# nekStab/nekStab_next

Hardware: AMD Instinct MI355X
Metric: Arnoldi-step GB/s (achieved HBM) + Ritz-value rel-err, N=1e8 m=128 (higher is better)
Workload: dtype f64

## Files before the change

### include/nekkrylov.h

```cpp
#ifndef NEKKRYLOV_H
#define NEKKRYLOV_H

#include <stddef.h>
#include <stdint.h>

#ifdef __cplusplus
extern "C" {
#endif

#define NKV_ABI_VERSION 3

#define NKV_TILE 4096
#define NKV_MAX_COLS 1024
#define NKV_ROT_MAX_OUT 256

#define NKV_OK 0
#define NKV_EINVAL 1
#define NKV_EHIP 2
#define NKV_ENAN 3
#define NKV_ESHAPE 4
#define NKV_ECALLBACK 5
#define NKV_EBREAKDOWN 6

#define NKV_TIME 0x1u
#define NKV_ACCUMULATE 0x2u
#define NKV_OVERWRITE 0x4u
#define NKV_NORM2 0x8u
#define NKV_TIME_DOT 0x10u
#define NKV_X_IS_LAST 0x20u
#define NKV_MGS2 0x40u
#define NKV_CHECK_BREAKDOWN 0x80u
#define NKV_MGS_ICWY 0x100u
#define NKV_MGS_LAGGED 0x200u
#define NKV_SFD_MONITOR 0x400u
#define NKV_TDF_STORE 0x800u
#define NKV_BF_IMAG 0x1000u
#define NKV_BF_PERTURBATION 0x2000u

typedef struct nkv_layout {
    int64_t n_v;
    int64_t n_p;
    int64_t sv;
    int64_t sp;
    int64_t ld;
    int32_t n_wf;
    int32_t rank0;
} nkv_layout;

int nkv_abi_version(void);
int nkv_layout_init(nkv_layout* L, int ldim, int lx1, int lx2, int64_t nelv, int64_t nelt, int n_scalars,
                    int ifpo, int rank0);
const char* nkv_last_error(void);
int nkv_device_info(int* device, int* cu_count, int64_t* hbm_bytes, char* name, int name_len);
size_t nkv_workspace_bytes(const nkv_layout* L, int max_cols);
int nkv_check_status(void* ws, void* stream);

int nkv_zero(const nkv_layout* L, double* x, unsigned flags, void* stream);
int nkv_copy(const nkv_layout* L, double* dst, const double* src, unsigned flags, void* stream);
int nkv_scal(const nkv_layout* L, double* x, double alpha, unsigned flags, void* stream);
int nkv_axpby(const nkv_layout* L, double* x, double alpha, const double* y, double beta,
// ... 14 lines not shown
                     double* f, double* nrm2_dev, void* ws, unsigned flags, void* stream);
int nkv_block_update_dot(const nkv_layout* L, const double* w, const double* Q, int j, const double* h_dev,
                         double* f, double* hout_dev, void* ws, unsigned flags, void* stream);
int nkv_arnoldi_finish(const nkv_layout* L, const double* f, const double* nrm2_dev, double* q_out,
                       int j, const double* h1_dev, const double* h2_dev, double* hcol_dev,
                       unsigned flags, void* stream);

int nkv_combine(const nkv_layout* L, const double* Q, int k, const double* y_dev, double* out, unsigned flags,
                void* stream);
int nkv_normalize_store(const nkv_layout* L, const double* f, const double* nrm2_dev, double* q_next,
                        double* beta_dev, unsigned flags, void* stream);
int nkv_mgs2_step(const nkv_layout* L, const double* w, const double* Q, int j, double* f, double* q_out,
                  double* hcol_dev, void* ws, unsigned flags, void* stream);
int nkv_axpy_dot(const nkv_layout* L, const double* w, double* f, const double* alpha_dev, const double* qa,
                 const double* qb, double* out_dev, void* ws, unsigned flags, void* stream);

int nkv_block_dot2(const nkv_layout* L, const double* w, const double* Q, int j, const double* x,
                   const double* y, double* h_dev, void* ws, unsigned flags, void* stream);
int nkv_dcgs2_coef(int m, const double* hq_dev, const double* hw_dev, const double* nrm_prev_dev, double* H_dev,
                   int64_t ldh, double* coef_dev, void* ws, void* stream);
int nkv_dcgs2_update(const nkv_layout* L, const double* w, const double* Q, int m, const double* coef_dev,
                     double* qj, const double* win, double* fout, double* nrm2_dev, void* ws, unsigned flags,
                     void* stream);

int nkv_mgs_icwy_solve(int j, double* G, int64_t ldg, const double* grow, const double* b, double* x,
                       void* stream);

int nkv_gkl_coef(int side, int m, const double* hq_dev, const double* hw_dev, double* M_dev, int64_t ldm,
                 double* A_self, double* r_self, const double* A_other, const double* r_other, int64_t lda,
                 double* coef_dev, void* ws, void* stream);

typedef int (*nkv_matvec_fn)(void* user, const double* x, double* y, void* stream);
typedef int (*nkv_allreduce_fn)(void* user, double* buf, int n, void* stream);
size_t nkv_arnoldi_scratch_doubles(int m);
int nkv_arnoldi_dcgs2(const nkv_layout* L, const double* w, double* Q, int mstart, int mend, double* H_dev,
                      int64_t ldh, double* f, double* scratch_dev, void* ws, nkv_matvec_fn matvec, void* mv_user,
                      nkv_allreduce_fn allreduce, void* ar_user, unsigned flags, void* stream);

int nkv_gmres_dcgs2(const nkv_layout* L, const double* w, double* Q, int kmax, double beta, double tol2,
                    double* H_dev, int64_t ldh, double* f, double* scratch_dev, void* ws, nkv_matvec_fn matvec,
                    void* mv_user, nkv_allreduce_fn allreduce, void* ar_user, double* res_hist, int* k_out,
                    unsigned flags, void* stream);

int nkv_update_hessenberg(const nkv_layout* L, const double* w, const double* Q, int j, double* f, double* q_out,
                          double* hcol_dev, double* scratch_dev, void* ws, nkv_allreduce_fn allreduce, void* ar_user,
                          unsigned flags, void* stream);
// ... 129 lines not shown
```

### nekstab_next_amd/_lib.py

```python
from __future__ import annotations

import ctypes
import os
from ctypes import CFUNCTYPE, POINTER, Structure, c_char_p, c_double, c_int, c_int32, c_int64, c_size_t, c_uint, c_uint64, c_void_p

import torch

_HERE = os.path.dirname(os.path.abspath(__file__))
LIB_PATH = os.path.join(_HERE, "libnekkrylov.so")

NKV_ABI_VERSION = 3
NKV_TILE = 4096
NKV_MAX_COLS = 1024
NKV_ROT_MAX_OUT = 256
NKV_GS_MAX_FIELDS = 64
NKV_OK, NKV_EINVAL, NKV_EHIP, NKV_ENAN, NKV_ESHAPE, NKV_ECALLBACK, NKV_EBREAKDOWN = 0, 1, 2, 3, 4, 5, 6
NKV_TIME = 0x1
NKV_ACCUMULATE = 0x2
NKV_OVERWRITE = 0x4
NKV_NORM2 = 0x8
NKV_TIME_DOT = 0x10
NKV_X_IS_LAST = 0x20
NKV_MGS2 = 0x40
NKV_MGS_ICWY = 0x100
NKV_MGS_LAGGED = 0x200
NKV_CHECK_BREAKDOWN = 0x80
NKV_SFD_MONITOR = 0x400
NKV_TDF_STORE = 0x800
NKV_BF_IMAG = 0x1000
NKV_BF_PERTURBATION = 0x2000
(NKV_VC_VORTICITY, NKV_VC_LAMBDA2, NKV_VC_Q, NKV_VC_DELTA, NKV_VC_SWIRLING, NKV_VC_OMEGA, NKV_VC_SYMMETRIC,
 NKV_VC_ASSYMETRIC, NKV_VC_LAMBDA_CI, NKV_VC_COUNT) = range(10)


class NkvError(RuntimeError):

    def __init__(self, code: int, where: str, msg: str):
        super().__init__(f"{where}: status {code}: {msg}")
        self.code = code


class NkvNaNError(NkvError, FloatingPointError):
    """NaN detected in a dot product (reference aborts: core/nek_vectors.f90:108-111)."""


class NkvBreakdownError(NkvError):
    """NKV_CHECK_BREAKDOWN: a one-call factorisation reached an invariant subspace (include/nekkrylov.h)."""


class nkv_layout(Structure):
    _fields_ = [
        ("n_v", c_int64),
        ("n_p", c_int64),
# ... 13 lines not shown
_SIGNATURES = {
    "nkv_abi_version": (c_int, []),
    "nkv_layout_init": (c_int, [_L, c_int, c_int, c_int, c_int64, c_int64, c_int, c_int, c_int]),
    "nkv_last_error": (c_char_p, []),
    "nkv_device_info": (c_int, [POINTER(c_int), POINTER(c_int), POINTER(c_int64), c_char_p, c_int]),
    "nkv_workspace_bytes": (c_size_t, [_L, c_int]),
    "nkv_check_status": (c_int, [_P, _P]),
    "nkv_zero": (c_int, [_L, _P, c_uint, _P]),
    "nkv_copy": (c_int, [_L, _P, _P, c_uint, _P]),
    "nkv_scal": (c_int, [_L, _P, c_double, c_uint, _P]),
    "nkv_axpby": (c_int, [_L, _P, c_double, _P, c_double, c_uint, _P]),
    "nkv_sub3": (c_int, [_L, _P, _P, _P, c_uint, _P]),
    "nkv_axpy_dev": (c_int, [_L, _P, _P, c_double, _P, c_uint, _P]),
    "nkv_normalize_dev": (c_int, [_L, _P, _P, _P, c_uint, _P]),
    "nkv_dot": (c_int, [_L, _P, _P, _P, _P, _P, c_uint, _P]),
    "nkv_block_dot": (c_int, [_L, _P, _P, c_int, _P, _P, _P, c_uint, _P]),
    "nkv_block_update": (c_int, [_L, _P, _P, c_int, _P, _P, _P, _P, c_uint, _P]),
    "nkv_block_update_dot": (c_int, [_L, _P, _P, c_int, _P, _P, _P, _P, c_uint, _P]),
    "nkv_arnoldi_finish": (c_int, [_L, _P, _P, _P, c_int, _P, _P, _P, c_uint, _P]),
    "nkv_block_dot2": (c_int, [_L, _P, _P, c_int, _P, _P, _P, _P, c_uint, _P]),
    "nkv_dcgs2_coef": (c_int, [c_int, _P, _P, _P, _P, c_int64, _P, _P, _P]),
    "nkv_mgs_icwy_solve": (c_int, [c_int, _P, c_int64, _P, _P, _P, _P]),
    "nkv_dcgs2_update": (c_int, [_L, _P, _P, c_int, _P, _P, _P, _P, _P, _P, c_uint, _P]),
    "nkv_arnoldi_scratch_doubles": (c_size_t, [c_int]),
    "nkv_arnoldi_dcgs2": (c_int, [_L, _P, _P, c_int, c_int, _P, c_int64, _P, _P, _P, MATVEC_FN, _P, ALLREDUCE_FN, _P,
                                  c_uint, _P]),
    "nkv_update_hessenberg": (c_int, [_L, _P, _P, c_int, _P, _P, _P, _P, _P, ALLREDUCE_FN, _P, c_uint, _P]),
    "nkv_gmres_dcgs2": (c_int, [_L, _P, _P, c_int, c_double, c_double, _P, c_int64, _P, _P, _P, MATVEC_FN, _P,
                                ALLREDUCE_FN, _P, _P, _P, c_uint, _P]),
    "nkv_arnoldi_factorization": (c_int, [_L, _P, _P, c_int, c_int, _P, c_int64, _P, _P, _P, MATVEC_FN, _P,
                                          ALLREDUCE_FN, _P, c_uint, _P]),
    "nkv_combine": (c_int, [_L, _P, c_int, _P, _P, c_uint, _P]),
    "nkv_normalize_store": (c_int, [_L, _P, _P, _P, _P, c_uint, _P]),
    "nkv_mgs2_step": (c_int, [_L, _P, _P, c_int, _P, _P, _P, _P, c_uint, _P]),
    "nkv_axpy_dot": (c_int, [_L, _P, _P, _P, _P, _P, _P, _P, c_uint, _P]),
    "nkv_rotate": (c_int, [_L, _P, c_int, _P, c_int, _P]),
    "nkv_rotate_cols": (c_int, [_L, _P, c_int, _P, c_int, c_int, _P]),
    "nkv_op_diag": (c_int, [_L, _P, _P, _P, c_double, _P]),
    "nkv_op_rot2": (c_int, [_L, _P, _P, _P, _P, _P, c_int, _P]),
    "nkv_op_cdiag": (c_int, [_L, _P, _P, _P, _P, c_int, _P]),
    "nkv_fill_hash": (c_int, [_L, _P, c_uint64, c_int64, c_int64, _P]),
    "nkv_mth_rand_add": (c_int, [_L, c_int, c_int, c_int, c_int64, _P, _P, _P, c_double, c_double, c_double, _P, _P]),
    "nkv_group_average": (c_int, [c_int64, _P, _P, _P, _P]),
    "nkv_symmetric_seed": (c_int, [_L, _P, _P, c_double, _P, _P, _P, _P]),
    "nkv_gs_pack": (c_int, [c_int, POINTER(c_void_p), c_int64, c_int64, _P, c_int64, _P, _P]),
    "nkv_gs_average": (c_int, [c_int, POINTER(c_void_p), c_int64, c_int64, _P, _P, _P, c_int64, c_int, _P]),
# ... 87 lines not shown
```

### nekstab_next_amd/arnoldi.py

```python
from __future__ import annotations

import numpy as np
import torch

from . import _lib
from ._lib import NKV_NORM2, NKV_TIME, NKV_TIME_DOT, NKV_X_IS_LAST
from .operators import LinearOperator
from .vector import Basis, NekContext, NekVector


class HessenbergDev:

    def __init__(self, ctx: NekContext, k: int):
        self.ctx, self.k = ctx, k
        self.t = torch.zeros((k, k + 1), dtype=torch.float64, device=ctx.device)

    def col_ptr(self, c: int) -> int:
        return self.t[c].data_ptr()

    def download(self) -> np.ndarray:
        return np.asfortranarray(self.t.detach().cpu().numpy().T)

    def upload(self, H: np.ndarray) -> None:
        self.t.copy_(torch.as_tensor(np.ascontiguousarray(np.asarray(H, dtype=np.float64).T)).to(self.ctx.device))
# ... 60 lines not shown
    elif mode == "mgs2":
        ctx.call("nkv_dot", w, f.ptr, Q.col_ptr(0), h1[0:1].data_ptr(), ws, tf, st)
        ctx.comm.allreduce_(h1[0:1])
        fl = NKV_TIME | (NKV_TIME_DOT if tf else 0)
        for p, h in enumerate((h1, h2)):
            for i in range(j):
                last = i + 1 == j
                qn = Q.col_ptr(i + 1) if not last else (Q.col_ptr(0) if p == 0 else None)
                out = h[i + 1:i + 2] if not last else (h2[0:1] if p == 0 else nrm)
                ctx.call("nkv_axpy_dot", w, f.ptr, h[i:i + 1].data_ptr(), Q.col_ptr(i), qn, out.data_ptr(), ws, fl,
                         st)
                ctx.comm.allreduce_(out)
    else:
        raise ValueError(f"unknown orthogonalisation mode {mode!r}")
    if ctx.timer:
        ctx.timer.begin("finish")
    ctx.call("nkv_arnoldi_finish", f.ptr, nrm.data_ptr(), out_ptr, j, h1.data_ptr(), h2.data_ptr(),
             hcol_ptr, 0, st)
    if ctx.timer:
        ctx.timer.end("finish", 16.0 * ctx.layout.N)


def _dcgs2_step(ctx: NekContext, Q: Basis, Hd: HessenbergDev, j: int, f: NekVector, first: bool,
                nrm2: torch.Tensor | None = None) -> None:
    w, ws, st = ctx.w.data_ptr(), ctx.ws.data_ptr(), ctx.stream
    lay, tm = ctx.layout, ctx.timer
    tf = NKV_TIME if ctx.time_in_dot else 0
    m = j - 1
    h = ctx.hd[: 2 * j]
    hp, cp = h.data_ptr(), ctx.coef.data_ptr()
    u = Q.col_ptr(m)
    if tm:
        tm.begin("block_dot2")
    ctx.call("nkv_block_dot2", w, Q.ptr, j, u, f.ptr, hp, ws, tf | NKV_X_IS_LAST, st)
    if tm:
        tm.end("block_dot2", 8.0 * ((j - 1) * lay.N_w + 2 * lay.N_w + lay.n_v))
    ctx.comm.allreduce_(h)
    nprev = None if first else (nrm2.data_ptr() if nrm2 is not None else hp + 8 * m)
    ctx.call_nl("nkv_dcgs2_coef", m, hp, hp + 8 * j, nprev, Hd.t.data_ptr(), Hd.k + 1, cp, ws, st)
    if tm:
        tm.begin("dcgs2_update")
    ctx.call("nkv_dcgs2_update", w, Q.ptr, m, cp, u, f.ptr, Q.col_ptr(j), None if nrm2 is None else nrm2.data_ptr(),
             ws, NKV_TIME | (NKV_TIME_DOT if tf else 0), st)
    if tm:
        tm.end("dcgs2_update", 8.0 * (m * lay.N + 4 * lay.N) + (0.0 if nrm2 is None else 8.0 * lay.n_v))
    if nrm2 is not None:
        ctx.comm.allreduce_(nrm2)


def _dcgs2_close(ctx: NekContext, Q: Basis, Hd: HessenbergDev, m: int) -> None:
    w, ws, st = ctx.w.data_ptr(), ctx.ws.data_ptr(), ctx.stream
    lay, tm = ctx.layout, ctx.timer
    tf = NKV_TIME if ctx.time_in_dot else 0
    h, coef = ctx.hd[: m + 1], ctx.coef
    u = Q.col_ptr(m)
    if tm:
        tm.begin("block_dot")
    ctx.call("nkv_block_dot", w, Q.ptr, m + 1, u, h.data_ptr(), ws, tf, st)
    if tm:
        tm.end("block_dot", 8.0 * ((m + 1) * lay.N_w + lay.N_w + lay.n_v))
    ctx.comm.allreduce_(h)
    ctx.call_nl("nkv_dcgs2_coef", m, h.data_ptr(), None, h.data_ptr() + 8 * m, Hd.t.data_ptr(), Hd.k + 1,
                coef.data_ptr(), ws, st)
    if tm:
        tm.begin("block_update")
    ctx.call("nkv_block_update", w, Q.ptr, m, h.data_ptr(), u, None, ws, NKV_TIME, st)
    if tm:
        tm.end("block_update", 8.0 * (m * lay.N + 2 * lay.N))
    ctx.call("nkv_normalize_dev", u, coef[2 * m + 3:].data_ptr(), None, 0, st)


def _icwy_gram(ctx: NekContext, Q: Basis, mstart: int) -> torch.Tensor:
    ldg = ctx.max_cols + 1
    G = getattr(ctx, "_icwy_G", None)
    if G is None:
        G = ctx._icwy_G = torch.zeros((ldg, ldg), dtype=torch.float64, device=ctx.device)
    w, ws, st = ctx.w.data_ptr(), ctx.ws.data_ptr(), ctx.stream
    tf = NKV_TIME if ctx.time_in_dot else 0
    for i in range(1, mstart - 1):
        ctx.call("nkv_block_dot", w, Q.ptr, i, Q.col_ptr(i), G[i].data_ptr(), ws, tf, st)
        ctx.comm.allreduce_(G[i, :i])
    return G


def _icwy_step(ctx: NekContext, Q: Basis, Hd: HessenbergDev, j: int, f: NekVector, G: torch.Tensor) -> None:
    w, ws, st = ctx.w.data_ptr(), ctx.ws.data_ptr(), ctx.stream
    lay, tm = ctx.layout, ctx.timer
    tf = NKV_TIME if ctx.time_in_dot else 0
    ldg = G.shape[1]
    h = ctx.hd[: 2 * j]
    hp, gp = h.data_ptr(), G.data_ptr()
    h1, h2, nrm = ctx.h1[:j], ctx.h2[:j], ctx.scal[3:4]
# ... 138 lines not shown


def _dcgs2_native(ctx: NekContext, op: LinearOperator, Q: Basis, Hd: HessenbergDev, mstart: int, mend: int,
                  f: NekVector, transpose: bool, entry: str = "nkv_arnoldi_dcgs2", flags: int = 0) -> None:
    lib = ctx.lib
    scratch = _native_scratch(ctx, mend)
    base, ld8, fptr = Q.ptr, 8 * ctx.layout.ld, f.ptr
    apply = op.rmatvec if transpose else op.matvec
    errors = []

    def matvec(_user, x, y, _stream):
        try:
            c, r = divmod((x or 0) - base, ld8)
            if r or not 0 <= c < Q.k or y != fptr:
                raise ValueError(f"{entry} matvec callback: x={x}, y={y} are not a basis column and f")
            apply(Q[c], f)
            return 0
        except BaseException as e:
            errors.append(e)
            return 1

    mv_c = _lib.MATVEC_FN(matvec)
    ar_c = _allreduce_callback(ctx, scratch, errors)
    rc = getattr(lib, entry)(ctx._Lp, ctx.w.data_ptr(), Q.ptr, int(mstart), int(mend), Hd.t.data_ptr(), Hd.k + 1,
                             fptr, scratch.data_ptr(), ctx.ws.data_ptr(), mv_c, None, ar_c, None,
                             (NKV_TIME_DOT if ctx.time_in_dot else 0) | flags, ctx.stream)
    if errors:
        raise errors[0]
    _lib.check(rc, entry)


def arnoldi_factorization(ctx: NekContext, op: LinearOperator, Q: Basis, Hd: HessenbergDev, mstart: int,
                          mend: int, f: NekVector | None = None, mode: str = "cgs2", transpose: bool = False,
                          on_step=None) -> None:
    if mend < mstart:
        return
    if Q.k < mend + 1:
        raise ValueError("basis too small")
    if f is None:
        f = ctx.vector()
    if mode == "dcgs2-native":
        if on_step is None:
            if mend > ctx.max_cols or mend + 1 > Hd.k + 1:
                raise ValueError(f"step {mend} exceeds max_cols {ctx.max_cols} / H size {Hd.k}")
            _dcgs2_native(ctx, op, Q, Hd, mstart, mend, f, transpose)
            return
        mode = "dcgs2"
    if mode == "dcgs2" and on_step is not None:
        if mend > ctx.max_cols or mend + 1 > Hd.k + 1:
            raise ValueError(f"step {mend} exceeds max_cols {ctx.max_cols} / H size {Hd.k}")
        for mstep in range(mstart, mend + 1):
            (op.rmatvec if transpose else op.matvec)(Q[mstep - 1], f)
            _dcgs2_step(ctx, Q, Hd, mstep, f, first=(mstep == mstart))
            if mstep > mstart:
                on_step(mstep - 1)
        _dcgs2_close(ctx, Q, Hd, mend)
        on_step(mend)
        return
    if mode == "mgs2-lagged-native":
        if on_step is None:
            if mend > ctx.max_cols or mend + 1 > Hd.k + 1:
                raise ValueError(f"step {mend} exceeds max_cols {ctx.max_cols} / H size {Hd.k}")
            _dcgs2_native(ctx, op, Q, Hd, mstart, mend, f, transpose, entry="nkv_arnoldi_factorization",
                          flags=_lib.NKV_MGS_LAGGED)
            return
        mode = "mgs2-lagged"
    if mode == "mgs2-lagged":
        if mend > ctx.max_cols or mend + 1 > Hd.k + 1:
            raise ValueError(f"step {mend} exceeds max_cols {ctx.max_cols} / H size {Hd.k}")
        _lagged_factorization(ctx, op, Q, Hd, mstart, mend, f, transpose, on_step)
        return
    if mode == "mgs2-icwy-native":
        if on_step is None:
            if mend > ctx.max_cols or mend + 1 > Hd.k + 1:
                raise ValueError(f"step {mend} exceeds max_cols {ctx.max_cols} / H size {Hd.k}")
            _dcgs2_native(ctx, op, Q, Hd, mstart, mend, f, transpose, entry="nkv_arnoldi_factorization",
                          flags=_lib.NKV_MGS_ICWY)
            return
        mode = "mgs2-icwy"
    if mode == "mgs2-icwy":
        if mend > ctx.max_cols or mend + 1 > Hd.k + 1:
            raise ValueError(f"step {mend} exceeds max_cols {ctx.max_cols} / H size {Hd.k}")
        G = _icwy_gram(ctx, Q, mstart)
        for mstep in range(mstart, mend + 1):
            (op.rmatvec if transpose else op.matvec)(Q[mstep - 1], f)
            _icwy_step(ctx, Q, Hd, mstep, f, G)
            if on_step is not None:
                on_step(mstep)
        return
    if mode in ("cgs2-native", "mgs2-native") and on_step is None:
        if mend > ctx.max_cols or mend + 1 > Hd.k + 1:
            raise ValueError(f"step {mend} exceeds max_cols {ctx.max_cols} / H size {Hd.k}")
        _dcgs2_native(ctx, op, Q, Hd, mstart, mend, f, transpose, entry="nkv_arnoldi_factorization",
                      flags=_lib.NKV_MGS2 if mode == "mgs2-native" else 0)
        return
    if mode == "dcgs2" and on_step is None:
        if mend > ctx.max_cols or mend + 1 > Hd.k + 1:
            raise ValueError(f"step {mend} exceeds max_cols {ctx.max_cols} / H size {Hd.k}")
        for mstep in range(mstart, mend + 1):
            (op.rmatvec if transpose else op.matvec)(Q[mstep - 1], f)
            _dcgs2_step(ctx, Q, Hd, mstep, f, first=(mstep == mstart))
        _dcgs2_close(ctx, Q, Hd, mend)
        return
    if mode == "dcgs2":
        mode = "cgs2"
    for mstep in range(mstart, mend + 1):
        x = Q[mstep - 1]
        (op.rmatvec if transpose else op.matvec)(x, f)
        update_hessenberg_matrix(ctx, Q, mstep, f, Hd, mode)
        if on_step is not None:
            on_step(mstep)


class FactorizationGraph:

    def __init__(self, ctx: NekContext, op: LinearOperator, Q: Basis, Hd: HessenbergDev, f: NekVector,
                 mode: str = "cgs2"):
        self.ctx, self.op, self.Q, self.Hd, self.f, self.mode = ctx, op, Q, Hd, f, mode
        self.graphs = {}

    HOST_SYNC_MODES = ("mgs2-lagged", "mgs2-lagged-native")

    def usable(self) -> bool:
        return self.ctx.comm.world == 1 and self.mode not in self.HOST_SYNC_MODES

# ... 17 lines not shown
```

### nekstab_next_amd/csrc/drivers.hip

```cpp
#include "nkv_internal.h"

#include <vector>

extern "C" {

static size_t icwy_scratch_doubles(int m) { return (size_t)(4 * (m + 1) + 2) + (size_t)(m + 1) * (size_t)(m + 1); }
size_t nkv_arnoldi_scratch_doubles(int m) {
    const size_t base = (size_t)(2 * (m + 1) + 4 * m + 16), icwy = icwy_scratch_doubles(m);
    return base > icwy ? base : icwy;
}

static constexpr double kBreakdownTol = 1e-8;

static int check_breakdown(const double* H_dev, int64_t ldh, int c0, int c1, void* ws, void* stream) {
    if (c0 < 0) c0 = 0;
    if (c1 <= c0) return NKV_OK;
    hipStream_t st = S(stream);
    const size_t n = (size_t)ldh * (size_t)(c1 - c0);
    double* h = static_cast<double*>(malloc(n * sizeof(double)));
    if (!h) return fail(NKV_EINVAL, "breakdown check: host allocation of %zu doubles failed", n);
    int flag = 0;
    hipError_t e = hipMemcpyAsync(h, H_dev + (int64_t)c0 * ldh, n * sizeof(double), hipMemcpyDeviceToHost, st);
    if (e == hipSuccess) e = hipMemcpyAsync(&flag, nan_flag_of(ws), sizeof(int), hipMemcpyDeviceToHost, st);
    if (e == hipSuccess) e = hipStreamSynchronize(st);
// ... 26 lines not shown
                      int64_t ldh, double* f, double* scratch_dev, void* ws, nkv_matvec_fn matvec, void* mv_user,
                      nkv_allreduce_fn allreduce, void* ar_user, unsigned flags, void* stream) {
    CHECK(check_layout(L));
    CHECK(check_ptr(Q, "Q"));
    CHECK(check_ptr(f, "f"));
    if (!matvec) return fail(NKV_EINVAL, "matvec callback is NULL");
    if (!H_dev || !scratch_dev) return fail(NKV_EINVAL, "H/scratch is NULL");
    if (mstart < 1 || mend > NKV_MAX_COLS) return fail(NKV_EINVAL, "steps %d..%d outside 1..%d", mstart, mend, NKV_MAX_COLS);
    if (mend < mstart) return NKV_OK;
    if (ldh < mend + 1) return fail(NKV_EINVAL, "ldh=%lld < mend+1=%d", (long long)ldh, mend + 1);
    const unsigned tf = (flags & NKV_TIME_DOT) ? NKV_TIME : 0u;
    double* hd = scratch_dev;
    double* coef = scratch_dev + 2 * (mend + 1);
    auto col = [L, Q](int c) { return Q + (int64_t)c * L->ld; };
    for (int j = mstart; j <= mend; ++j) {
        const int m = j - 1;
        double* u = col(m);
        int rc = matvec(mv_user, u, f, stream);
        if (rc != 0) return fail(NKV_ECALLBACK, "matvec callback returned %d at step %d", rc, j);
        CHECK(nkv_block_dot2(L, w, Q, j, u, f, hd, ws, tf | NKV_X_IS_LAST, stream));
        if (allreduce && (rc = allreduce(ar_user, hd, 2 * j, stream)) != 0)
            return fail(NKV_ECALLBACK, "allreduce callback returned %d at step %d", rc, j);
        CHECK(nkv_dcgs2_coef(m, hd, hd + j, j == mstart ? nullptr : hd + m, H_dev, ldh, coef, ws, stream));
        CHECK(nkv_dcgs2_update(L, w, Q, m, coef, u, f, col(j), nullptr, ws, NKV_TIME, stream));
    }
    const int m = mend;
    double* u = col(m);
    CHECK(nkv_block_dot(L, w, Q, m + 1, u, hd, ws, tf, stream));
    if (allreduce) {
        const int rc = allreduce(ar_user, hd, m + 1, stream);
        if (rc != 0) return fail(NKV_ECALLBACK, "allreduce callback returned %d (closing step)", rc);
    }
    CHECK(nkv_dcgs2_coef(m, hd, nullptr, hd + m, H_dev, ldh, coef, ws, stream));
    CHECK(nkv_block_update(L, w, Q, m, hd, u, nullptr, ws, NKV_TIME, stream));
    CHECK(nkv_normalize_dev(L, u, coef + 2 * m + 3, nullptr, 0, stream));
    return (flags & NKV_CHECK_BREAKDOWN) ? check_breakdown(H_dev, ldh, mstart - 1, mend, ws, stream) : NKV_OK;
}

int nkv_gmres_dcgs2(const nkv_layout* L, const double* w, double* Q, int kmax, double beta, double tol2,
                    double* H_dev, int64_t ldh, double* f, double* scratch_dev, void* ws, nkv_matvec_fn matvec,
                    void* mv_user, nkv_allreduce_fn allreduce, void* ar_user, double* res_hist, int* k_out,
                    unsigned flags, void* stream) {
    CHECK(check_layout(L));
    CHECK(check_ptr(Q, "Q"));
    CHECK(check_ptr(f, "f"));
    CHECK(check_ptr(w, "w"));
    CHECK(check_ptr(ws, "ws"));
    if (!matvec) return fail(NKV_EINVAL, "matvec callback is NULL");
    if (!H_dev || !scratch_dev || !res_hist || !k_out) return fail(NKV_EINVAL, "H/scratch/res_hist/k_out is NULL");
    if (kmax < 1 || kmax + 1 > NKV_MAX_COLS) return fail(NKV_EINVAL, "kmax=%d outside 1..%d", kmax, NKV_MAX_COLS - 1);
    if (ldh < kmax + 1) return fail(NKV_EINVAL, "ldh=%lld < kmax+1=%d", (long long)ldh, kmax + 1);
    hipStream_t st = S(stream);
    const unsigned tf = (flags & NKV_TIME_DOT) ? NKV_TIME : 0u;
    double* hd = scratch_dev;
    double* coef = scratch_dev + 2 * (kmax + 1);
    double* nrm2 = scratch_dev + nkv_arnoldi_scratch_doubles(kmax) - 1;
    double* host = nullptr;
    if (hipHostMalloc(reinterpret_cast<void**>(&host), sizeof(double) * (size_t)(4 * (kmax + 2)),
// ... 317 lines not shown
```

### nekstab_next_amd/csrc/gram_schmidt.hip

```cpp
#include "nkv_internal.h"

namespace {

template <bool OVERWRITE, bool NORM, int kPairs>
__global__ __launch_bounds__(kThreads) void k_block_update(const double* __restrict__ Q, int64_t ld,
                                                           int j, const double* __restrict__ h,
                                                           double* __restrict__ f,
                                                           const double* __restrict__ w, int64_t sv,
                                                           int tiles_per_field, int tiles_w,
                                                           int tiles_total, int64_t time_off,
                                                           int do_time,
                                                           double* __restrict__ partials, int t_lo,
                                                           int acc_part) {
    constexpr int kTile = kThreads * kPairs * 2;
    __shared__ double lds4[4];
    if (do_time && blockIdx.x == 0 && threadIdx.x < 64) {
        double s = 0.0;
        for (int c = threadIdx.x; c < j; c += 64) s = fma(Q[time_off + (int64_t)c * ld], h[c], s);
        s = wave_sum(s);
        if (threadIdx.x == 0) f[time_off] = OVERWRITE ? s : f[time_off] - s;
    }
    double nrm = 0.0;
    for (int t = t_lo + blockIdx.x; t < tiles_total; t += gridDim.x) {
        const int64_t r0 = (int64_t)t * kTile + 2 * threadIdx.x;
        double2 acc[kPairs];
#pragma unroll
        for (int k = 0; k < kPairs; ++k) {
            if (OVERWRITE) acc[k] = make_double2(0.0, 0.0);
            else acc[k] = ld2(f + r0 + k * 2 * kThreads);
        }
        const double* qb = Q + r0;
        int c = 0;
        for (; c + 4 <= j; c += 4) {
            double2 q[4][kPairs];
#pragma unroll
            for (int u = 0; u < 4; ++u)
#pragma unroll
                for (int k = 0; k < kPairs; ++k) q[u][k] = ldq(qb + (int64_t)(c + u) * ld + k * 2 * kThreads);
#pragma unroll
            for (int u = 0; u < 4; ++u) {
                const double hc = OVERWRITE ? h[c + u] : -h[c + u];
#pragma unroll
                for (int k = 0; k < kPairs; ++k) {
                    acc[k].x = fma(hc, q[u][k].x, acc[k].x);
                    acc[k].y = fma(hc, q[u][k].y, acc[k].y);
                }
            }
        }
        for (; c < j; ++c) {
            const double hc = OVERWRITE ? h[c] : -h[c];
#pragma unroll
            for (int k = 0; k < kPairs; ++k) {
                const double2 q = ldq(qb + (int64_t)c * ld + k * 2 * kThreads);
                acc[k].x = fma(hc, q.x, acc[k].x);
                acc[k].y = fma(hc, q.y, acc[k].y);
            }
        }
#pragma unroll
        for (int k = 0; k < kPairs; ++k) st2(f + r0 + k * 2 * kThreads, acc[k]);
        if (NORM && t < tiles_w) {
            const int64_t wr = r0 - (int64_t)(t / tiles_per_field) * sv;
#pragma unroll
            for (int k = 0; k < kPairs; ++k) {
                const double2 wv = ld2(w + wr + k * 2 * kThreads);
                nrm = fma(wv.x * acc[k].x, acc[k].x, nrm);
                nrm = fma(wv.y * acc[k].y, acc[k].y, nrm);
            }
        }
    }
    if (NORM) {
        nrm = block_sum(nrm, lds4);
        if (threadIdx.x == 0) partials[blockIdx.x] = acc_part ? partials[blockIdx.x] + nrm : nrm;
    }
}

constexpr int kFuseRows = 128;

template <int NW, int CPW>
__global__ __launch_bounds__(NW * 64) void k_update_dot(const double* __restrict__ Q, int64_t ld, int j,
// ... 466 lines not shown
    for (int u = blockIdx.x; u < n_units; u += gridDim.x) {
        if (u < tiles_per_field) {
            double2 wv[kPairs];
#pragma unroll
            for (int k = 0; k < kPairs; ++k) wv[k] = ld2(w + (int64_t)u * kTile + 2 * threadIdx.x + k * 2 * kThreads);
            for (int fi = 0; fi < n_wf; ++fi) {
                dcgs2_tile<kPairs>(Q, ld, m, a, x, rinv, yc, sc, qj, win, f,
                                   (int64_t)(fi * tiles_per_field + u) * kTile + 2 * threadIdx.x, af);
#pragma unroll
                for (int k = 0; k < kPairs; ++k) {
                    nrm = fma(wv[k].x * af[k].x, af[k].x, nrm);
                    nrm = fma(wv[k].y * af[k].y, af[k].y, nrm);
                }
            }
        } else {
            dcgs2_tile<kPairs>(Q, ld, m, a, x, rinv, yc, sc, qj, win, f,
                               (int64_t)(tiles_w + u - tiles_per_field) * kTile + 2 * threadIdx.x, af);
        }
    }
    nrm = block_sum(nrm, lds4);
    if (threadIdx.x == 0) partials[blockIdx.x] = nrm;
}

template <int P>
int launch_block_update_p(const nkv_layout* L, const double* w, const double* Q, int j, const double* h_dev,
                          double* f, double* part, unsigned flags, hipStream_t st, int* g_out) {
    constexpr int kTile = kThreads * P * 2;
    const bool over = (flags & NKV_OVERWRITE) != 0;
    const bool norm = (flags & NKV_NORM2) != 0;
    const int tpf = (int)(L->sv / kTile);
    const int tiles_w = tpf * L->n_wf;
    const int tiles_total = (int)(rows_of(L) / kTile);
    const int gmax = j <= NKV_UPD_SMALL_J ? 4 * kMaxBlocks : kMaxBlocks;
    int g = tiles_total < gmax ? tiles_total : gmax;
    if (g < 1) g = 1;
    *g_out = g;
    const int64_t T = rows_of(L);
    const int dt = (flags & NKV_TIME) ? 1 : 0;
    auto kern = over ? (norm ? k_block_update<true, true, P> : k_block_update<true, false, P>)
                     : (norm ? k_block_update<false, true, P> : k_block_update<false, false, P>);
    const int64_t b = (int64_t)NKV_UPD_ROUNDS * g;
    const int band = (NKV_UPD_ROUNDS <= 0 || b >= tiles_total || tiles_total < 2 * b) ? (tiles_total > 0 ? tiles_total : 1)
                                                                                        : (int)b;
    for (int lo = 0; lo == 0 || lo < tiles_total; lo += band) {
        const int hi = lo + band < tiles_total ? lo + band : tiles_total;
        const int gb = lo == 0 ? g : (g < hi - lo ? g : hi - lo);
        hipLaunchKernelGGL(kern, dim3(gb), dim3(kThreads), 0, st, Q, L->ld, j, h_dev, f, w, L->sv, tpf, tiles_w, hi, T,
                           lo == 0 ? dt : 0, part, lo, lo == 0 ? 0 : 1);
        NKV_LAUNCHED();
    }
    return NKV_OK;
}

inline int band_tiles(int tiles_total, int g) {
    if (NKV_DC_ROUNDS <= 0) return tiles_total > 0 ? tiles_total : 1;
    const int64_t b = (int64_t)NKV_DC_ROUNDS * g;
    return (b >= tiles_total || tiles_total < 2 * b) ? (tiles_total > 0 ? tiles_total : 1) : (int)b;
}

__global__ __launch_bounds__(kThreads) void k_mgs_icwy_solve(int j, double* __restrict__ G, int64_t ldg,
                                                             const double* __restrict__ grow,
                                                             const double* b, double* x) {
    extern __shared__ double xs[];
    for (int i = threadIdx.x; i < j; i += kThreads) xs[i] = b[i];
    if (grow)
        for (int k = threadIdx.x; k < j - 1; k += kThreads) G[(int64_t)(j - 1) * ldg + k] = grow[k];
    for (int k = 0; k + 1 < j; ++k) {
        __syncthreads();
        const double xk = xs[k];
        for (int i = k + 1 + threadIdx.x; i < j; i += kThreads) {
            const double g = (grow && i == j - 1) ? grow[k] : G[(int64_t)i * ldg + k];
// ... 225 lines not shown
    const int dt = (flags & NKV_TIME) ? 1 : 0;
    double* part = partials_of(ws);
    auto kern = large ? (nrm2_dev ? k_dcgs2_update<NKV_DC_PAIRS, true> : k_dcgs2_update<NKV_DC_PAIRS, false>)
                      : (nrm2_dev ? k_dcgs2_update<NKV_PAIRS_SMALL, true> : k_dcgs2_update<NKV_PAIRS_SMALL, false>);
    if (!nrm2_dev) {
        const int band = band_tiles(tiles_total, g);
        for (int lo = 0; lo == 0 || lo < tiles_total; lo += band) {
            const int hi = lo + band < tiles_total ? lo + band : tiles_total;
            const int gb = g < hi - lo ? g : (hi - lo > 0 ? hi - lo : 1);
            hipLaunchKernelGGL(kern, dim3(gb), dim3(kThreads), 0, st, Q, L->ld, m, coef_dev, qj, win, fout, w, L->sv,
                               tpf, tiles_w, tiles_total, T, lo == 0 ? dt : 0, part, lo, hi);
            NKV_LAUNCHED();
        }
        return NKV_OK;
    }
    hipLaunchKernelGGL(kern, dim3(g), dim3(kThreads), 0, st, Q, L->ld, m, coef_dev, qj, win, fout, w, L->sv, tpf,
                       tiles_w, tiles_total, T, dt, part, 0, tiles_total);
    NKV_LAUNCHED();
    const bool tdot = (flags & NKV_TIME_DOT) && L->rank0;
    CHECK(launch_reduce_cols(1, part, g, nrm2_dev, tdot ? fout + T : nullptr, (int64_t)0, tdot ? fout + T : nullptr, nullptr, 1 << 30, nan_flag_of(ws), st));
    return NKV_OK;
}

int nkv_combine(const nkv_layout* L, const double* Q, int k, const double* y_dev, double* out, unsigned flags,
                void* stream) {
    return nkv_block_update(L, nullptr, Q, k, y_dev, out, nullptr, nullptr,
                            (flags & ~(unsigned)NKV_NORM2) | NKV_OVERWRITE, stream);
}

}
```

### nekstab_next_amd/csrc/nkv_internal.h

```cpp
#pragma once

#include <hip/hip_runtime.h>

#include <cmath>
#include <cstdarg>
#include <cstdio>
#include <cstdlib>
#include <cstring>

#include "nekkrylov.h"

#ifndef NKV_PAIRS
#define NKV_PAIRS 8
#endif
#ifndef NKV_PAIRS_SMALL
#define NKV_PAIRS_SMALL 4
#endif
#ifndef NKV_SMALL_TILES
#define NKV_SMALL_TILES 2048
#endif
#ifndef NKV_COLU
#define NKV_COLU 4
#endif
#ifndef NKV_NT
// ... 28 lines not shown
#endif
#ifndef NKV_STREAM_UNR
#define NKV_STREAM_UNR 4
#endif
#ifndef NKV_DC_G
#define NKV_DC_G 768
#endif
#ifndef NKV_UPD_ROUNDS
#define NKV_UPD_ROUNDS 2
#endif
#ifndef NKV_AXD_ROUNDS
#define NKV_AXD_ROUNDS 0
#endif
#ifndef NKV_UPD_SMALL_J
#define NKV_UPD_SMALL_J 2
#endif
#ifndef NKV_FUSE_SMALL_J
#define NKV_FUSE_SMALL_J 12
#endif
static_assert(NKV_FUSE_SMALL_J >= 0 && NKV_FUSE_SMALL_J <= 16,
              "the 4-wave fused pass instantiates at most 16 columns (NKV_FUSE(4, 4))");
#ifndef NKV_FUSE_ROUNDS
#define NKV_FUSE_ROUNDS 0
#endif
#ifndef NKV_DC_ROUNDS
#define NKV_DC_ROUNDS 2
#endif
#ifndef NKV_STREAM_ROUNDS
#define NKV_STREAM_ROUNDS 2
#endif
#ifndef NKV_D2_MAXB
#define NKV_D2_MAXB 256
#endif
#ifndef NKV_D2_SMALL_B
#define NKV_D2_SMALL_B 512
#endif
#ifndef NKV_DOT_SMALL_B
#define NKV_DOT_SMALL_B 512
#endif
#ifndef NKV_D2_FIELDLOOP
#define NKV_D2_FIELDLOOP 1
#endif
#ifndef NKV_D2_U
#define NKV_D2_U 2
#endif
#ifndef NKV_D2_PAIRS
// ... 288 lines not shown
```

Before: 6845.

## Fuse closing block dot into last DCGS2 update and fold normalization into block update

For the final Arnoldi step, a new kernel performs the DCGS2 update and computes the closing weighted dot products of the new vector against all basis columns in the same pass. This removes the separate block_dot read of Q. The closing block update now applies the normalization scale inline, which drops a separate normalize pass over the output vector. In exchange it adds a new templated kernel with LDS cross-wave reductions and many instantiations, plus a fallback path for large sizes.

```diff
diff --git a/include/nekkrylov.h b/include/nekkrylov.h
--- a/include/nekkrylov.h
+++ b/include/nekkrylov.h
@@ -36,6 +36,7 @@
 #define NKV_TDF_STORE 0x800u
 #define NKV_BF_IMAG 0x1000u
 #define NKV_BF_PERTURBATION 0x2000u
+#define NKV_DOTS_UNFUSED 0x4000u
 
 typedef struct nkv_layout {
     int64_t n_v;
@@ -96,6 +97,12 @@
 int nkv_dcgs2_update(const nkv_layout* L, const double* w, const double* Q, int m, const double* coef_dev,
                      double* qj, const double* win, double* fout, double* nrm2_dev, void* ws, unsigned flags,
                      void* stream);
+int nkv_dcgs2_update_dots(const nkv_layout* L, const double* w, const double* Q, int m, const double* coef_dev,
+                          double* qj, const double* win, double* fout, double* dots_dev, void* ws, unsigned flags,
+                          void* stream);
+int nkv_dcgs2_dots_fused(const nkv_layout* L, int m, unsigned flags);
+int nkv_block_update_scaled(const nkv_layout* L, const double* Q, int j, const double* h_dev, double* f,
+                            const double* nrm2_dev, unsigned flags, void* stream);
 
 int nkv_mgs_icwy_solve(int j, double* G, int64_t ldg, const double* grow, const double* b, double* x,
                        void* stream);
diff --git a/nekstab_next_amd/_lib.py b/nekstab_next_amd/_lib.py
--- a/nekstab_next_amd/_lib.py
+++ b/nekstab_next_amd/_lib.py
@@ -29,6 +29,7 @@
 NKV_TDF_STORE = 0x800
 NKV_BF_IMAG = 0x1000
 NKV_BF_PERTURBATION = 0x2000
+NKV_DOTS_UNFUSED = 0x4000
 (NKV_VC_VORTICITY, NKV_VC_LAMBDA2, NKV_VC_Q, NKV_VC_DELTA, NKV_VC_SWIRLING, NKV_VC_OMEGA, NKV_VC_SYMMETRIC,
  NKV_VC_ASSYMETRIC, NKV_VC_LAMBDA_CI, NKV_VC_COUNT) = range(10)
 
@@ -88,6 +89,9 @@
     "nkv_dcgs2_coef": (c_int, [c_int, _P, _P, _P, _P, c_int64, _P, _P, _P]),
     "nkv_mgs_icwy_solve": (c_int, [c_int, _P, c_int64, _P, _P, _P, _P]),
     "nkv_dcgs2_update": (c_int, [_L, _P, _P, c_int, _P, _P, _P, _P, _P, _P, c_uint, _P]),
+    "nkv_dcgs2_update_dots": (c_int, [_L, _P, _P, c_int, _P, _P, _P, _P, _P, _P, c_uint, _P]),
+    "nkv_dcgs2_dots_fused": (c_int, [_L, c_int, c_uint]),
+    "nkv_block_update_scaled": (c_int, [_L, _P, c_int, _P, _P, _P, c_uint, _P]),
     "nkv_arnoldi_scratch_doubles": (c_size_t, [c_int]),
     "nkv_arnoldi_dcgs2": (c_int, [_L, _P, _P, c_int, c_int, _P, c_int64, _P, _P, _P, MATVEC_FN, _P, ALLREDUCE_FN, _P,
                                   c_uint, _P]),
diff --git a/nekstab_next_amd/arnoldi.py b/nekstab_next_amd/arnoldi.py
--- a/nekstab_next_amd/arnoldi.py
+++ b/nekstab_next_amd/arnoldi.py
@@ -106,7 +106,7 @@
 
 
 def _dcgs2_step(ctx: NekContext, Q: Basis, Hd: HessenbergDev, j: int, f: NekVector, first: bool,
-                nrm2: torch.Tensor | None = None) -> None:
+                nrm2: torch.Tensor | None = None, last: bool = False) -> None:
     w, ws, st = ctx.w.data_ptr(), ctx.ws.data_ptr(), ctx.stream
     lay, tm = ctx.layout, ctx.timer
     tf = NKV_TIME if ctx.time_in_dot else 0
@@ -124,6 +124,15 @@
     ctx.call_nl("nkv_dcgs2_coef", m, hp, hp + 8 * j, nprev, Hd.t.data_ptr(), Hd.k + 1, cp, ws, st)
     if tm:
         tm.begin("dcgs2_update")
+    if last:
+        if nrm2 is not None:
+            raise ValueError("the fused closing dots and the fused norm are exclusive")
+        unfused = _lib.NKV_DOTS_UNFUSED if getattr(ctx, "dcgs2_unfused", False) else 0
+        ctx.call("nkv_dcgs2_update_dots", w, Q.ptr, m, cp, u, f.ptr, Q.col_ptr(j), ctx.hd.data_ptr(), ws,
+                 NKV_TIME | (NKV_TIME_DOT if tf else 0) | unfused, st)
+        if tm:
+            tm.end("dcgs2_update", 8.0 * (m * lay.N + 4 * lay.N) + 8.0 * lay.n_v)
+        return
     ctx.call("nkv_dcgs2_update", w, Q.ptr, m, cp, u, f.ptr, Q.col_ptr(j), None if nrm2 is None else nrm2.data_ptr(),
              ws, NKV_TIME | (NKV_TIME_DOT if tf else 0), st)
     if tm:
@@ -132,26 +141,31 @@
         ctx.comm.allreduce_(nrm2)
 
 
-def _dcgs2_close(ctx: NekContext, Q: Basis, Hd: HessenbergDev, m: int) -> None:
+def _dcgs2_close(ctx: NekContext, Q: Basis, Hd: HessenbergDev, m: int, dots_ready: bool = False) -> None:
     w, ws, st = ctx.w.data_ptr(), ctx.ws.data_ptr(), ctx.stream
     lay, tm = ctx.layout, ctx.timer
     tf = NKV_TIME if ctx.time_in_dot else 0
     h, coef = ctx.hd[: m + 1], ctx.coef
     u = Q.col_ptr(m)
-    if tm:
-        tm.begin("block_dot")
-    ctx.call("nkv_block_dot", w, Q.ptr, m + 1, u, h.data_ptr(), ws, tf, st)
-    if tm:
-        tm.end("block_dot", 8.0 * ((m + 1) * lay.N_w + lay.N_w + lay.n_v))
+    if not dots_ready:
+        if tm:
+            tm.begin("block_dot")
+        ctx.call("nkv_block_dot", w, Q.ptr, m + 1, u, h.data_ptr(), ws, tf, st)
+        if tm:
+            tm.end("block_dot", 8.0 * ((m + 1) * lay.N_w + lay.N_w + lay.n_v))
     ctx.comm.allreduce_(h)
     ctx.call_nl("nkv_dcgs2_coef", m, h.data_ptr(), None, h.data_ptr() + 8 * m, Hd.t.data_ptr(), Hd.k + 1,
                 coef.data_ptr(), ws, st)
     if tm:
         tm.begin("block_update")
-    ctx.call("nkv_block_update", w, Q.ptr, m, h.data_ptr(), u, None, ws, NKV_TIME, st)
+    if dots_ready:
+        ctx.call("nkv_block_update_scaled", Q.ptr, m, h.data_ptr(), u, coef[2 * m + 3:].data_ptr(), NKV_TIME, st)
+    else:
+        ctx.call("nkv_block_update", w, Q.ptr, m, h.data_ptr(), u, None, ws, NKV_TIME, st)
     if tm:
         tm.end("block_update", 8.0 * (m * lay.N + 2 * lay.N))
-    ctx.call("nkv_normalize_dev", u, coef[2 * m + 3:].data_ptr(), None, 0, st)
+    if not dots_ready:
+        ctx.call("nkv_normalize_dev", u, coef[2 * m + 3:].data_ptr(), None, 0, st)
 
 
 def _icwy_gram(ctx: NekContext, Q: Basis, mstart: int) -> torch.Tensor:
@@ -336,9 +350,10 @@
 
     mv_c = _lib.MATVEC_FN(matvec)
     ar_c = _allreduce_callback(ctx, scratch, errors)
+    unfused = _lib.NKV_DOTS_UNFUSED if entry == "nkv_arnoldi_dcgs2" and getattr(ctx, "dcgs2_unfused", False) else 0
     rc = getattr(lib, entry)(ctx._Lp, ctx.w.data_ptr(), Q.ptr, int(mstart), int(mend), Hd.t.data_ptr(), Hd.k + 1,
                              fptr, scratch.data_ptr(), ctx.ws.data_ptr(), mv_c, None, ar_c, None,
-                             (NKV_TIME_DOT if ctx.time_in_dot else 0) | flags, ctx.stream)
+                             (NKV_TIME_DOT if ctx.time_in_dot else 0) | flags | unfused, ctx.stream)
     if errors:
         raise errors[0]
     _lib.check(rc, entry)
@@ -365,10 +380,10 @@
             raise ValueError(f"step {mend} exceeds max_cols {ctx.max_cols} / H size {Hd.k}")
         for mstep in range(mstart, mend + 1):
             (op.rmatvec if transpose else op.matvec)(Q[mstep - 1], f)
-            _dcgs2_step(ctx, Q, Hd, mstep, f, first=(mstep == mstart))
+            _dcgs2_step(ctx, Q, Hd, mstep, f, first=(mstep == mstart), last=(mstep == mend))
             if mstep > mstart:
                 on_step(mstep - 1)
-        _dcgs2_close(ctx, Q, Hd, mend)
+        _dcgs2_close(ctx, Q, Hd, mend, dots_ready=True)
         on_step(mend)
         return
     if mode == "mgs2-lagged-native":
@@ -413,8 +428,8 @@
             raise ValueError(f"step {mend} exceeds max_cols {ctx.max_cols} / H size {Hd.k}")
         for mstep in range(mstart, mend + 1):
             (op.rmatvec if transpose else op.matvec)(Q[mstep - 1], f)
-            _dcgs2_step(ctx, Q, Hd, mstep, f, first=(mstep == mstart))
-        _dcgs2_close(ctx, Q, Hd, mend)
+            _dcgs2_step(ctx, Q, Hd, mstep, f, first=(mstep == mstart), last=(mstep == mend))
+        _dcgs2_close(ctx, Q, Hd, mend, dots_ready=True)
         return
     if mode == "dcgs2":
         mode = "cgs2"
diff --git a/nekstab_next_amd/csrc/drivers.hip b/nekstab_next_amd/csrc/drivers.hip
--- a/nekstab_next_amd/csrc/drivers.hip
+++ b/nekstab_next_amd/csrc/drivers.hip
@@ -72,18 +72,19 @@
         if (allreduce && (rc = allreduce(ar_user, hd, 2 * j, stream)) != 0)
             return fail(NKV_ECALLBACK, "allreduce callback returned %d at step %d", rc, j);
         CHECK(nkv_dcgs2_coef(m, hd, hd + j, j == mstart ? nullptr : hd + m, H_dev, ldh, coef, ws, stream));
-        CHECK(nkv_dcgs2_update(L, w, Q, m, coef, u, f, col(j), nullptr, ws, NKV_TIME, stream));
+        if (j < mend) CHECK(nkv_dcgs2_update(L, w, Q, m, coef, u, f, col(j), nullptr, ws, NKV_TIME, stream));
+        else
+            CHECK(nkv_dcgs2_update_dots(L, w, Q, m, coef, u, f, col(j), hd, ws,
+                                        NKV_TIME | (flags & (NKV_TIME_DOT | NKV_DOTS_UNFUSED)), stream));
     }
     const int m = mend;
     double* u = col(m);
-    CHECK(nkv_block_dot(L, w, Q, m + 1, u, hd, ws, tf, stream));
     if (allreduce) {
         const int rc = allreduce(ar_user, hd, m + 1, stream);
         if (rc != 0) return fail(NKV_ECALLBACK, "allreduce callback returned %d (closing step)", rc);
     }
     CHECK(nkv_dcgs2_coef(m, hd, nullptr, hd + m, H_dev, ldh, coef, ws, stream));
-    CHECK(nkv_block_update(L, w, Q, m, hd, u, nullptr, ws, NKV_TIME, stream));
-    CHECK(nkv_normalize_dev(L, u, coef + 2 * m + 3, nullptr, 0, stream));
+    CHECK(nkv_block_update_scaled(L, Q, m, hd, u, coef + 2 * m + 3, NKV_TIME, stream));
     return (flags & NKV_CHECK_BREAKDOWN) ? check_breakdown(H_dev, ldh, mstart - 1, mend, ws, stream) : NKV_OK;
 }
 
diff --git a/nekstab_next_amd/csrc/gram_schmidt.hip b/nekstab_next_amd/csrc/gram_schmidt.hip
--- a/nekstab_next_amd/csrc/gram_schmidt.hip
+++ b/nekstab_next_amd/csrc/gram_schmidt.hip
@@ -2,7 +2,7 @@
 
 namespace {
 
-template <bool OVERWRITE, bool NORM, int kPairs>
+template <bool OVERWRITE, bool NORM, int kPairs, bool SCALE = false>
 __global__ __launch_bounds__(kThreads) void k_block_update(const double* __restrict__ Q, int64_t ld,
                                                            int j, const double* __restrict__ h,
                                                            double* __restrict__ f,
@@ -11,14 +11,21 @@
                                                            int tiles_total, int64_t time_off,
                                                            int do_time,
                                                            double* __restrict__ partials, int t_lo,
-                                                           int acc_part) {
+                                                           int acc_part, const double* __restrict__ scale2) {
     constexpr int kTile = kThreads * kPairs * 2;
     __shared__ double lds4[4];
+    double inv = 1.0;
+    if (SCALE) inv = 1.0 / sqrt(scale2[0]);
     if (do_time && blockIdx.x == 0 && threadIdx.x < 64) {
         double s = 0.0;
-        for (int c = threadIdx.x; c < j; c += 64) s = fma(Q[time_off + (int64_t)c * ld], h[c], s);
-        s = wave_sum(s);
-        if (threadIdx.x == 0) f[time_off] = OVERWRITE ? s : f[time_off] - s;
+        if (do_time & 1) {
+            for (int c = threadIdx.x; c < j; c += 64) s = fma(Q[time_off + (int64_t)c * ld], h[c], s);
+            s = wave_sum(s);
+        }
+        if (threadIdx.x == 0) {
+            const double v = OVERWRITE ? s : f[time_off] - s;
+            f[time_off] = SCALE ? v * inv : v;
+        }
     }
     double nrm = 0.0;
     for (int t = t_lo + blockIdx.x; t < tiles_total; t += gridDim.x) {
@@ -55,6 +62,10 @@
                 acc[k].x = fma(hc, q.x, acc[k].x);
                 acc[k].y = fma(hc, q.y, acc[k].y);
             }
+        }
+        if (SCALE) {
+#pragma unroll
+            for (int k = 0; k < kPairs; ++k) acc[k] = make_double2(acc[k].x * inv, acc[k].y * inv);
         }
 #pragma unroll
         for (int k = 0; k < kPairs; ++k) st2(f + r0 + k * 2 * kThreads, acc[k]);
@@ -567,9 +578,114 @@
     if (threadIdx.x == 0) partials[blockIdx.x] = nrm;
 }
 
+template <int NW, int CPW>
+__global__ __launch_bounds__(NW * 64) void k_dcgs2_update_dots(const double* __restrict__ Q, int64_t ld, int m,
+                                                                const double* __restrict__ coef,
+                                                                double* __restrict__ qj,
+                                                                const double* __restrict__ win,
+                                                                double* __restrict__ f,
+                                                                const double* __restrict__ w, int64_t sv,
+                                                                int64_t tiles_per_field, int64_t tiles_w,
+                                                                int64_t tiles_total, int64_t time_off,
+                                                                int do_time, double* __restrict__ partials, int B) {
+    __shared__ double2 part_a[2][NW][64];
+    __shared__ double2 part_x[2][NW][64];
+    const int wv = __builtin_amdgcn_readfirstlane(threadIdx.x >> 6);
+    const int lane = threadIdx.x & 63;
+    const double* x = coef;
+    const double* a = coef + 2 * m + 5;
+    const double rinv = coef[2 * m + 1], yc = coef[2 * m + 2], sc = coef[2 * m + 4];
+    const double wsc = sc * rinv;
+    if (do_time && blockIdx.x == 0 && wv == 0) {
+        double s1 = 0.0, s2 = 0.0;
+        for (int c = lane; c < m; c += 64) {
+            const double qt = Q[time_off + (int64_t)c * ld];
+            s1 = fma(qt, a[c], s1);
+            s2 = fma(qt, x[c], s2);
+        }
+        s1 = wave_sum(s1);
+        s2 = wave_sum(s2);
+        if (lane == 0) {
+            const double qb = (qj[time_off] * sc - s1) * rinv;
+            qj[time_off] = qb;
+            f[time_off] = win[time_off] * wsc - s2 - qb * yc;
+        }
+    }
+    const double* qcol[CPW];
+    double ac[CPW], xc[CPW];
+#pragma unroll
+    for (int i = 0; i < CPW; ++i) {
+        const int c = wv + NW * i;
+        qcol[i] = Q + (int64_t)(c < m ? c : 0) * ld;
+        ac[i] = c < m ? a[c] : 0.0;
+        xc[i] = c < m ? x[c] : 0.0;
+    }
+    double acc[CPW];
+#pragma unroll
+    for (int i = 0; i < CPW; ++i) acc[i] = 0.0;
+    double acc_q = 0.0, acc_f = 0.0;
+    int buf = 0;
+    double2 q[CPW];
+    for (int64_t t = blockIdx.x; t < tiles_total; t += gridDim.x, buf ^= 1) {
+        const uint32_t r = (uint32_t)(t * kFuseRows) + 2u * lane;
+        const uint32_t rb = r * 8u;
+#pragma unroll
+        for (int i = 0; i < CPW - 1; ++i) q[i] = ldq(at_b(qcol[i], rb));
+        q[CPW - 1] = (wv + NW * (CPW - 1) < m) ? ldq(at_b(qcol[CPW - 1], rb)) : make_double2(0.0, 0.0);
+        double2 sa = make_double2(0.0, 0.0), sx = make_double2(0.0, 0.0);
+#pragma unroll
+        for (int i = 0; i < CPW; ++i) {
+            sa.x = fma(ac[i], q[i].x, sa.x);
+            sa.y = fma(ac[i], q[i].y, sa.y);
+            sx.x = fma(xc[i], q[i].x, sx.x);
+            sx.y = fma(xc[i], q[i].y, sx.y);
+        }
+        const double2 uv = ld2(at_b(qj, rb));
+        const double2 fv = ld2(at_b(win, rb));
+        const bool weighted = t < tiles_w;
+        const double2 ww = weighted ? ld2(at_b(w, (r - (uint32_t)((t / tiles_per_field) * sv)) * 8u)) : make_double2(0.0, 0.0);
+        part_a[buf][wv][lane] = sa;
+        part_x[buf][wv][lane] = sx;
+        __syncthreads();
+        double2 ta = part_a[buf][0][lane], tx = part_x[buf][0][lane];
+#pragma unroll
+        for (int k = 1; k < NW; ++k) {
+            const double2 pa = part_a[buf][k][lane], px = part_x[buf][k][lane];
+            ta.x += pa.x;
+            ta.y += pa.y;
+            tx.x += px.x;
+            tx.y += px.y;
+        }
+        const double2 qb = make_double2((uv.x * sc - ta.x) * rinv, (uv.y * sc - ta.y) * rinv);
+        const double2 f1 = make_double2(fma(-yc, qb.x, fv.x * wsc - tx.x), fma(-yc, qb.y, fv.y * wsc - tx.y));
+        if (wv == 0) st2s(const_cast<double*>(at_b(qj, rb)), qb);
+        if (wv == 1) st2s(const_cast<double*>(at_b(f, rb)), f1);
+        if (weighted) {
+            const double wa = ww.x * f1.x, wb = ww.y * f1.y;
+#pragma unroll
+            for (int i = 0; i < CPW; ++i) acc[i] = fma(q[i].y, wb, fma(q[i].x, wa, acc[i]));
+            acc_q = fma(qb.y, wb, fma(qb.x, wa, acc_q));
+            acc_f = fma(f1.y, wb, fma(f1.x, wa, acc_f));
+        }
+    }
+#pragma unroll
+    for (int i = 0; i < CPW; ++i) {
+        const int c = wv + NW * i;
+        const double v = wave_sum(acc[i]);
+        if (lane == 0 && c < m) partials[(int64_t)c * B + blockIdx.x] = v;
+    }
+    acc_q = wave_sum(acc_q);
+    acc_f = wave_sum(acc_f);
+    if (wv == 0 && lane == 0) {
+        partials[(int64_t)m * B + blockIdx.x] = acc_q;
+        partials[(int64_t)(m + 1) * B + blockIdx.x] = acc_f;
+    }
+}
+
 template <int P>
 int launch_block_update_p(const nkv_layout* L, const double* w, const double* Q, int j, const double* h_dev,
-                          double* f, double* part, unsigned flags, hipStream_t st, int* g_out) {
+                          double* f, double* part, unsigned flags, hipStream_t st, int* g_out,
+                          const double* scale2 = nullptr) {
     constexpr int kTile = kThreads * P * 2;
     const bool over = (flags & NKV_OVERWRITE) != 0;
     const bool norm = (flags & NKV_NORM2) != 0;
@@ -584,6 +700,8 @@
     const int dt = (flags & NKV_TIME) ? 1 : 0;
     auto kern = over ? (norm ? k_block_update<true, true, P> : k_block_update<true, false, P>)
                      : (norm ? k_block_update<false, true, P> : k_block_update<false, false, P>);
+    if (scale2) kern = k_block_update<false, false, P, true>;
+    const int st_bit = scale2 ? 2 : 0;
     const int64_t b = (int64_t)NKV_UPD_ROUNDS * g;
     const int band = (NKV_UPD_ROUNDS <= 0 || b >= tiles_total || tiles_total < 2 * b) ? (tiles_total > 0 ? tiles_total : 1)
                                                                                         : (int)b;
@@ -591,7 +709,7 @@
         const int hi = lo + band < tiles_total ? lo + band : tiles_total;
         const int gb = lo == 0 ? g : (g < hi - lo ? g : hi - lo);
         hipLaunchKernelGGL(kern, dim3(gb), dim3(kThreads), 0, st, Q, L->ld, j, h_dev, f, w, L->sv, tpf, tiles_w, hi, T,
-                           lo == 0 ? dt : 0, part, lo, lo == 0 ? 0 : 1);
+                           lo == 0 ? (dt | st_bit) : 0, part, lo, lo == 0 ? 0 : 1, scale2);
         NKV_LAUNCHED();
     }
     return NKV_OK;
@@ -863,6 +981,103 @@
     return NKV_OK;
 }
 
+int nkv_dcgs2_dots_fused(const nkv_layout* L, int m, unsigned flags) {
+    if (!L || m < 0 || m > 256 || (flags & NKV_DOTS_UNFUSED)) return 0;
+    return rows_of(L) < ((int64_t)1 << 29) ? 1 : 0;
+}
+
+int nkv_dcgs2_update_dots(const nkv_layout* L, const double* w, const double* Q, int m, const double* coef_dev,
+                          double* qj, const double* win, double* fout, double* dots_dev, void* ws, unsigned flags,
+                          void* stream) {
+    CHECK(check_layout(L));
+    CHECK(check_ptr(w, "w"));
+    CHECK(check_ptr(Q, "Q"));
+    CHECK(check_ptr(qj, "qj"));
+    CHECK(check_ptr(win, "win"));
+    CHECK(check_ptr(fout, "fout"));
+    CHECK(check_ptr(ws, "ws"));
+    if (m < 0 || m + 2 > NKV_MAX_COLS) return fail(NKV_EINVAL, "m=%d outside 0..%d", m, NKV_MAX_COLS - 2);
+    if (!coef_dev || !dots_dev) return fail(NKV_EINVAL, "coef/dots is NULL");
+    if (qj != Q + (int64_t)m * L->ld || fout != qj + L->ld)
+        return fail(NKV_EINVAL, "dcgs2_update_dots: qj / fout are not columns m / m+1 of Q");
+    const unsigned dot_flags = (flags & NKV_TIME_DOT) ? NKV_TIME : 0u;
+    hipStream_t st = S(stream);
+    if (!nkv_dcgs2_dots_fused(L, m, flags)) {
+        CHECK(nkv_dcgs2_update(L, w, Q, m, coef_dev, qj, win, fout, nullptr, ws, flags & NKV_TIME, stream));
+        return launch_block_dot(L, w, Q, L->ld, m + 2, fout, dots_dev, ws, dot_flags, st);
+    }
+    const int64_t rows = rows_of(L);
+    const int64_t tiles_total = rows / kFuseRows;
+    const int64_t tpf = L->sv / kFuseRows;
+    const int64_t tiles_w = tpf * L->n_wf;
+    const int64_t gcap = (m >= NKV_FUSE_MID_LO && m <= NKV_FUSE_MID_HI) ? NKV_FUSE_G_MID : NKV_FUSE_G;
+    int64_t g = tiles_total < gcap ? tiles_total : gcap;
+    if (g < 1) g = 1;
+    const int B = (int)g;
+    const int dt = (flags & NKV_TIME) ? 1 : 0;
+    double* part = partials_of(ws);
+#define NKV_DCD(NW, CPW)                                                                                          \
+    hipLaunchKernelGGL((k_dcgs2_update_dots<NW, CPW>), dim3((unsigned)g), dim3(NW * 64), 0, st, Q, L->ld, m,      \
+                       coef_dev, qj, win, fout, w, L->sv, tpf, tiles_w, tiles_total, rows, dt, part, B)
+#define NKV_DCD_CASES(NW)                                                                                         \
+    switch (cpw) {                                                                                                \
+        case 1: NKV_DCD(NW, 1); break;                                                                            \
+        case 2: NKV_DCD(NW, 2); break;                                                                            \
+        case 3: NKV_DCD(NW, 3); break;                                                                            \
+        case 4: NKV_DCD(NW, 4); break;                                                                            \
+        case 5: NKV_DCD(NW, 5); break;                                                                            \
+        case 6: NKV_DCD(NW, 6); break;                                                                            \
+        case 7: NKV_DCD(NW, 7); break;                                                                            \
+        case 8: NKV_DCD(NW, 8); break;                                                                            \
+        case 9: NKV_DCD(NW, 9); break;                                                                            \
+        case 10: NKV_DCD(NW, 10); break;                                                                          \
+        case 11: NKV_DCD(NW, 11); break;                                                                          \
+        case 12: NKV_DCD(NW, 12); break;                                                                          \
+        case 13: NKV_DCD(NW, 13); break;                                                                          \
+        case 14: NKV_DCD(NW, 14); break;                                                                          \
+        case 15: NKV_DCD(NW, 15); break;                                                                          \
+        default: NKV_DCD(NW, 16); break;                                                                          \
+    }
+    constexpr int NW = NKV_FUSE_NW;
+    constexpr int kWide = NKV_DCD_WIDE_M < NW * 16 ? NKV_DCD_WIDE_M : NW * 16;
+    if (m <= NKV_FUSE_SMALL_J) {
+        switch ((m + 3) / 4) {
+            case 0:
+            case 1: NKV_DCD(4, 1); break;
+            case 2: NKV_DCD(4, 2); break;
+            case 3: NKV_DCD(4, 3); break;
+            default: NKV_DCD(4, 4); break;
+        }
+    } else if (m <= kWide) {
+        const int cpw = (m + NW - 1) / NW;
+        NKV_DCD_CASES(NW)
+    } else {
+        const int cpw = (m + 15) / 16;
+        NKV_DCD_CASES(16)
+    }
+#undef NKV_DCD_CASES
+#undef NKV_DCD
+    NKV_LAUNCHED();
+    const bool tdot = (flags & NKV_TIME_DOT) && L->rank0;
+    CHECK(launch_reduce_cols(m + 2, part, B, dots_dev, tdot ? Q + rows : nullptr, L->ld, tdot ? fout + rows : nullptr,
+                             nullptr, 1 << 30, nan_flag_of(ws), st));
+    return NKV_OK;
+}
+
+int nkv_block_update_scaled(const nkv_layout* L, const double* Q, int j, const double* h_dev, double* f,
+                            const double* nrm2_dev, unsigned flags, void* stream) {
+    CHECK(check_layout(L));
+    CHECK(check_ptr(Q, "Q"));
+    CHECK(check_ptr(f, "f"));
+    if (!h_dev || !nrm2_dev) return fail(NKV_EINVAL, "h_dev/nrm2_dev is NULL");
+    if (j < 0) return fail(NKV_EINVAL, "j=%d < 0", j);
+    int g = 1;
+    const unsigned uf = flags & NKV_TIME;
+    if (use_large_tiles(L))
+        return launch_block_update_p<NKV_PAIRS>(L, nullptr, Q, j, h_dev, f, nullptr, uf, S(stream), &g, nrm2_dev);
+    return launch_block_update_p<NKV_PAIRS_SMALL>(L, nullptr, Q, j, h_dev, f, nullptr, uf, S(stream), &g, nrm2_dev);
+}
+
 int nkv_combine(const nkv_layout* L, const double* Q, int k, const double* y_dev, double* out, unsigned flags,
                 void* stream) {
     return nkv_block_update(L, nullptr, Q, k, y_dev, out, nullptr, nullptr,
diff --git a/nekstab_next_amd/csrc/nkv_internal.h b/nekstab_next_amd/csrc/nkv_internal.h
--- a/nekstab_next_amd/csrc/nkv_internal.h
+++ b/nekstab_next_amd/csrc/nkv_internal.h
@@ -74,6 +74,9 @@
               "the 4-wave fused pass instantiates at most 16 columns (NKV_FUSE(4, 4))");
 #ifndef NKV_FUSE_ROUNDS
 #define NKV_FUSE_ROUNDS 0
+#endif
+#ifndef NKV_DCD_WIDE_M
+#define NKV_DCD_WIDE_M 128
 #endif
 #ifndef NKV_DC_ROUNDS
 #define NKV_DC_ROUNDS 2
```

New measurement: 6795. Within noise of the previous version (-0.7%).
